# kokkos/kokkos-kernels

Measured on AMD Instinct MI355X. Metric: SpMV GFLOP/s (CSR, 27-pt 3-D FE Laplacian, fp64), higher is better.
Workload: dtype f64

## Files before the change

### kokkos-kernels_amd/csrc/kk_spmv.hip

```cpp
#include "kk_common.h"
#include "kk_scan.h"
#include <new>
#include <cstring>
#include <climits>

#include "kk_spmv_plan.h"

namespace kk {

template <class OffT, class AT, class YT, int LPR>
__global__ __launch_bounds__(kBlock) void spmv_vector_kernel(int64_t nrows, const OffT* __restrict__ row_map,
                                                             const int32_t* __restrict__ entries,
                                                             const AT* __restrict__ values, const YT* __restrict__ x,
                                                             YT* __restrict__ y, YT alpha, YT beta, int remap) {
  constexpr int RPB = kBlock / LPR;
  const int64_t wg  = remap ? xcd_remap(blockIdx.x, gridDim.x) : (int64_t)blockIdx.x;
  const int64_t row = wg * RPB + threadIdx.x / LPR;
  const int lane    = threadIdx.x % LPR;
  YT sum            = YT(0);
  if (row < nrows) {
    const OffT s = row_map[row], e = row_map[row + 1];
    for (OffT j = s + lane; j < e; j += LPR) sum += (YT)values[j] * x[entries[j]];
  }
  sum = group_sum(sum, LPR);
// ... 134 lines not shown
  uint16_t* out = wcode + s + (int64_t)t * NPT;
  if constexpr (NPT % 8 == 0) {
    KK_UNROLL
    for (int k = 0; k < NPT; k += 8) {
      kk_u32x4 v;
      v[0] = code[k] | (code[k + 1] << 16); v[1] = code[k + 2] | (code[k + 3] << 16);
      v[2] = code[k + 4] | (code[k + 5] << 16); v[3] = code[k + 6] | (code[k + 7] << 16);
      *reinterpret_cast<kk_u32x4*>(out + k) = v;
    }
  } else {
    KK_UNROLL
    for (int k = 0; k < NPT; k += 2) *reinterpret_cast<unsigned*>(out + k) = code[k] | (code[k + 1] << 16);
  }
  if (t == 0) {
    int off = 0;
    for (int w = 0; w < kWinCount; ++w) { s_off[w] = off; off += 64 * s_nch[w]; }
    s_off[kWinCount] = off;
    constexpr int CAP = TILE < kWinChunks * 64 ? TILE : kWinChunks * 64;
    const int mode = (off > CAP || !allow_stage) ? kTileCodes : kTileStaged;
    tinfo[b] = mode;
  }
  __syncthreads();
  int32_t* meta = wmeta + b * kWinMeta;
  if (t < kWinCount) { meta[t] = s_base[t]; meta[kWinCount + t] = s_off[t]; }
  if (t < kWinChunks) {
    const int slot = t * 64;
    int col = -1;
    for (int w = 0; w < kWinCount; ++w) if (slot >= s_off[w] && slot < s_off[w] + 64 * s_nch[w]) col = s_base[w] + (slot - s_off[w]);
    meta[2 * kWinCount + t] = col;
  }
}

constexpr int kPatSeg = 8, kPatLen = 32, kPatRec = 8, kPatTab = kPatRec + 4 * kPatSeg, kPatW = kPatTab + kPatSeg * kPatLen / 2;

template <class OffT, int NPT>
__global__ __launch_bounds__(kBlock) void pat_build_kernel(int64_t nnz, const OffT* __restrict__ row_map,
                                                           const int32_t* __restrict__ blk_info,
                                                           const uint16_t* __restrict__ wcode, const int32_t* __restrict__ wmeta,
                                                           int32_t* __restrict__ tinfo, int32_t* __restrict__ pmeta) {
  constexpr int TILE = kBlock * NPT, STEPS = NPT / 2, SPAN = kBlock * 2;
  __shared__ unsigned short s_slot[TILE];
  __shared__ unsigned char s_head[TILE + 2];
  __shared__ int s_segq[kPatSeg];
  __shared__ int s_nseg, s_bad, s_chunks;
  const int t = threadIdx.x;
  const int64_t b = blockIdx.x, s = b * TILE;
  int32_t* out = pmeta + b * kPatW;
  if ((tinfo[b] & 3) != kTileStaged) return;
  if (t == 0) { s_nseg = 0; s_bad = (s + TILE <= nnz) ? 0 : 1; s_chunks = 0; }
  __syncthreads();
  const int ldsoff = wmeta[b * kWinMeta + kWinCount + (t & (kWinCount - 1))];
  KK_UNROLL
  for (int k = 0; k < STEPS; ++k) {
    KK_UNROLL
    for (int j = 0; j < 2; ++j) {
      const unsigned code = wcode[s + (int64_t)t * NPT + 2 * k + j];
      const int off = __shfl(ldsoff, (int)(code >> kWinBits), 64);
      s_slot[k * SPAN + 2 * t + j] = (unsigned short)(off + (int)(code & ((1u << kWinBits) - 1)));
    }
  }
  if (t < kWinChunks && wmeta[b * kWinMeta + 2 * kWinCount + t] >= 0) atomicAdd(&s_chunks, 1);
  const int32_t info0 = blk_info[b], info1 = blk_info[b + 1];
  const int64_t ra = info0 & 0x7fffffff, rb = info1 & 0x7fffffff;
  const int has_head = (info0 >> 31) & 1;
  const int64_t nv = (rb - ra) + has_head;
  __syncthreads();
// ... 2 lines not shown
    const int64_t r  = ra + q - has_head;
    const int64_t rs = (int64_t)row_map[r] - s, re = (int64_t)row_map[r + 1] - s, L = re - rs;
    bool head = true;
    if (L < 1 || L > kPatLen) atomicOr(&s_bad, 1);
    else if (q > 0) {
      const int64_t ps = (int64_t)row_map[r - 1] - s;
      if (rs - ps == L) {
        head = false;
        for (int k = 0; k < (int)L; ++k) {
          const int64_t i0 = ps + k, i1 = rs + k;
          if (i0 >= 0 && i1 < TILE && (int)s_slot[i1] != (int)s_slot[i0] + 1) head = true;
        }
      }
    }
    s_head[q] = head ? 1 : 0;
    if (head) { const int idx = atomicAdd(&s_nseg, 1); if (idx < kPatSeg) s_segq[idx] = (int)q; }
  }
  __syncthreads();
  const int nseg = s_nseg;
  if (s_bad || nseg > kPatSeg || nseg < 1) return;
  if (t == 0) {
    for (int a = 1; a < nseg; ++a) { const int v = s_segq[a]; int c = a - 1; while (c >= 0 && s_segq[c] > v) { s_segq[c + 1] = s_segq[c]; --c; } s_segq[c + 1] = v; }
  }
  __syncthreads();
  if (t < kPatSeg) {
    int sb = INT_MAX, rs32 = 0, L32 = 1; float M = 1.0f;
    if (t < nseg) {
      const int64_t r  = ra + s_segq[t] - has_head;
      const int64_t rs = (int64_t)row_map[r] - s, L = (int64_t)row_map[r + 1] - s - rs;
      sb = rs > 0 ? (int)rs : 0; rs32 = (int)rs; L32 = (int)L;
      M  = 1.0f / (float)L;
    }
    if (t >= 1) out[t] = sb;
    out[kPatRec + 4 * t + 0] = sb; out[kPatRec + 4 * t + 1] = -rs32; out[kPatRec + 4 * t + 2] = L32; out[kPatRec + 4 * t + 3] = __float_as_int(M);
  }
  if (t == 0) { out[0] = nseg; tinfo[b] = kTilePattern; }
  if (t < kPatSeg * kPatLen) {
    const int g = t / kPatLen, k = t % kPatLen;
    int val = 0;
    if (g < nseg) {
      const int q = s_segq[g];
      const int64_t r  = ra + q - has_head;
      const int64_t rs = (int64_t)row_map[r] - s, re = (int64_t)row_map[r + 1] - s;
      if (k < re - rs) {
        const int64_t i = rs + k;
        if (i >= 0 && i < TILE) val = (int)s_slot[i];
        else if (i < 0 && q + 1 < nv && !s_head[q + 1] && re + k < TILE) val = (int)s_slot[re + k] - 1;
      }
    }
    reinterpret_cast<short*>(out + kPatTab)[t] = (short)val;
  }
}

template <class OffT, int NPT>
__global__ __launch_bounds__(kBlock) void pat_direct_kernel(int64_t nnz, const OffT* __restrict__ row_map, const int32_t* __restrict__ entries,
                                                            const int32_t* __restrict__ blk_info, int32_t* __restrict__ wmeta,
                                                            int32_t* __restrict__ tinfo, int32_t* __restrict__ pmeta) {
  constexpr int TILE = kBlock * NPT, NI = kPatSeg * kPatLen;
  static_assert(NI == kBlock, "one interval per work-item");
  __shared__ int s_col[TILE];
  __shared__ int s_segq[kPatSeg];
  __shared__ int s_lo[NI], s_hi[NI];
  __shared__ int s_base[kWinCount], s_nch[kWinCount], s_off[kWinCount + 1];
  __shared__ int s_nseg, s_bad;
  const int t = threadIdx.x, lane = t & 63, wave = t >> 6;
  const int64_t b = blockIdx.x, s = b * TILE;
  int32_t* out = pmeta + b * kPatW;
// ... 89 lines not shown
      bool unc = false;
      KK_UNROLL
      for (int u = 0; u < NI / 64; ++u) unc |= ((long long)ihi[u] >= bound);
      failed = __ballot(unc) != 0ull;
      if (!failed && lane == 0) {
        for (int q = wn; q < kWinCount; ++q) { s_base[q] = q ? s_base[q - 1] : 0; s_nch[q] = 0; }
        int off = 0;
        for (int w = 0; w < kWinCount; ++w) { s_off[w] = off; off += 64 * s_nch[w]; }
        s_off[kWinCount] = off;
      }
    }
    if (lane == 0 && failed) s_bad = 1;
  }
  __syncthreads();
  constexpr int CAP = TILE < kWinChunks * 64 ? TILE : kWinChunks * 64;
  if (s_bad || s_off[kWinCount] > CAP || s_off[kWinCount] > TILE - kPatW) { if (t == 0) tinfo[b] = kTilePlain; return; }
  int32_t* meta = wmeta + b * kWinMeta;
  if (t < kWinCount) { meta[t] = s_base[t]; meta[kWinCount + t] = s_off[t]; }
  if (t < kWinChunks) {
    const int slot = t * 64;
    int col = -1;
    for (int w = 0; w < kWinCount; ++w) if (slot >= s_off[w] && slot < s_off[w] + 64 * s_nch[w]) col = s_base[w] + (slot - s_off[w]);
    meta[2 * kWinCount + t] = col;
  }
  if (t < kPatSeg) {
    int sb = INT_MAX, rs32 = 0, L32 = 1; float M = 1.0f;
    if (t < nseg) {
      const int64_t r  = ra + s_segq[t] - has_head;
      const int64_t rs = (int64_t)row_map[r] - s, L = (int64_t)row_map[r + 1] - s - rs;
      sb = rs > 0 ? (int)rs : 0; rs32 = (int)rs; L32 = (int)L;
      M  = 1.0f / (float)L;
    }
    if (t >= 1) out[t] = sb;
    out[kPatRec + 4 * t + 0] = sb; out[kPatRec + 4 * t + 1] = -rs32; out[kPatRec + 4 * t + 2] = L32; out[kPatRec + 4 * t + 3] = __float_as_int(M);
  }
  if (t == 0) { out[0] = nseg; tinfo[b] = kTilePattern; }
  {
    int val = 0;
    if (csrc >= 0) {
      for (int w = 0; w < kWinCount; ++w) if (s_nch[w] > 0 && csrc >= s_base[w] && csrc < s_base[w] + 64 * s_nch[w]) val = s_off[w] + (csrc - s_base[w]);
      val += cadj;
    }
    reinterpret_cast<short*>(out + kPatTab)[t] = (short)val;
  }
}

__global__ __launch_bounds__(kBlock) void tile_mode_hist_kernel(int64_t nblocks, const int32_t* __restrict__ tinfo, int* __restrict__ counts) {
  __shared__ int s_c[4];
  const int t = threadIdx.x;
  if (t < 4) s_c[t] = 0;
  __syncthreads();
  const int64_t b = (int64_t)blockIdx.x * kBlock + t;
  const int mode = b < nblocks ? (tinfo[b] & 3) : -1;
  for (int m = 0; m < 4; ++m) {
    const int c = __popcll(__ballot(mode == m));
    if ((t & 63) == 0 && c) atomicAdd(&s_c[m], c);
  }
  __syncthreads();
  if (t < 4 && s_c[t]) atomicAdd(counts + t, s_c[t]);
}

__global__ void code_flag_kernel(int64_t nblocks, int32_t* __restrict__ tinfo, int32_t* __restrict__ flag, int use_pat) {
  const int64_t b = (int64_t)blockIdx.x * blockDim.x + threadIdx.x;
  if (b > nblocks) return;
  if (b == nblocks) { flag[b] = 0; return; }
  int mode = tinfo[b] & 3;
  if (mode == kTilePattern && !use_pat) { mode = kTileStaged; tinfo[b] = mode; }
// ... 224 lines not shown
  YT x0[STEPS], x1[STEPS];
  KK_UNROLL
  for (int k = 0; k < STEPS; ++k) {
    x0[k] = (FULL || c0[k] >= 0) ? x[FULL ? c0[k] : (c0[k] >= 0 ? c0[k] : 0)] : YT(0);
    x1[k] = (FULL || c1[k] >= 0) ? x[FULL ? c1[k] : (c1[k] >= 0 ? c1[k] : 0)] : YT(0);
  }
  KK_UNROLL
  for (int k = 0; k < STEPS; ++k) {
    const int li = k * SPAN + t * 2;
    prod[li]     = (YT)v0[k] * x0[k];
    prod[li + 1] = (YT)v1[k] * x1[k];
  }
}

template <class YT> __device__ __forceinline__ YT strided_lds_sum(const YT* prod, int i0, int i1, int lane, int G) {
  YT s0 = YT(0), s1 = YT(0), s2 = YT(0), s3 = YT(0);
  int i = i0 + lane;
  const int G2 = 2 * G, G3 = 3 * G, G4 = 4 * G;
  for (; i + G3 < i1; i += G4) {
    const YT a = prod[i], b = prod[i + G], c = prod[i + G2], d = prod[i + G3];
    s0 += a; s1 += b; s2 += c; s3 += d;
  }
  for (; i < i1; i += G) s0 += prod[i];
  return (s0 + s1) + (s2 + s3);
}

template <class OffT, class AT, class YT, int NPT, int MODE>
__global__ __launch_bounds__(kBlock) void spmv_stream3_kernel(int64_t nnz, const OffT* __restrict__ row_map,
                                                              const int32_t* __restrict__ entries,
                                                              const AT* __restrict__ values, const YT* __restrict__ x,
                                                              YT* __restrict__ y, YT alpha, YT beta,
                                                              const int32_t* __restrict__ blk_info,
                                                              YT* __restrict__ carry_head, YT* __restrict__ carry_tail,
                                                              int remap, const int32_t* __restrict__ list,
                                                              const int32_t* __restrict__ tinfo,
                                                              const uint16_t* __restrict__ wcode,
                                                              const int32_t* __restrict__ wmeta, int64_t ncols,
                                                              const int32_t* __restrict__ pmeta KK_ABL_PARAM) {
  constexpr int TILE  = kBlock * NPT;
  constexpr int STEPS = NPT / 2;
  __shared__ YT prod[TILE];
  constexpr bool NT = false;
  const int t       = threadIdx.x;
  const int64_t pos = xcd_order(blockIdx.x, gridDim.x, remap);
  const int64_t b   = list ? (int64_t)list[pos] : pos;
  const int64_t s = b * TILE;
  const bool full = (s + TILE <= nnz);
  const int64_t e = full ? s + TILE : nnz;

  const int32_t info0 = blk_info[b], info1 = blk_info[b + 1];
  const uint16_t* wtile = nullptr;
  if (MODE == kTileCodes || MODE == kTileStaged) wtile = wcode + (int64_t)((unsigned)tinfo[b] >> 2) * TILE;

  AT v0[STEPS], v1[STEPS];
  int c0[STEPS], c1[STEPS];
  if (MODE >= kTileStaged) {
  } else if (MODE == kTileCodes) {
    if (full) load_tile_win<AT, STEPS, true>(values, wtile, wmeta, b, s, e, t, v0, v1, c0, c1);
    else      load_tile_win<AT, STEPS, false>(values, wtile, wmeta, b, s, e, t, v0, v1, c0, c1);
  } else {
    if (full) load_tile<AT, STEPS, NT, true>(values, entries, s, e, t, v0, v1, c0, c1);
    else      load_tile<AT, STEPS, NT, false>(values, entries, s, e, t, v0, v1, c0, c1);
  }

  const int64_t ra    = info0 & 0x7fffffff;
  const int64_t rb    = info1 & 0x7fffffff;
  const int has_head  = (info0 >> 31) & 1;
  const int64_t nv    = (rb - ra) + has_head;
  int G = 1;
  while (G < kWave && nv * (G * 2) <= kBlock) G *= 2;
  const int lane = t & (G - 1), grp = t / G, ngrp = kBlock / G;
  bool valid = grp < nv;
  int64_t r  = ra + grp - has_head;
  int64_t rs = 0, re = 0;
  if (valid) {
    if (KK_ABL(16)) { rs = s + (int64_t)grp * 27; re = rs + 27; }
    else { rs = (int64_t)row_map[r]; re = (int64_t)row_map[r + 1]; }
  }
  YT yold = YT(0);
  if (beta != YT(0) && valid && lane == 0 && r >= 0) yold = y[r];

  if (MODE == kTilePattern) {
    stage_products_win<AT, YT, STEPS, true, NT, true>(values, wtile, wmeta, x, ncols, prod, b, s, e, t, pmeta);
  } else if (MODE == kTileStaged) {
    if (full) stage_products_win<AT, YT, STEPS, true, NT, false>(values, wtile, wmeta, x, ncols, prod, b, s, e, t, nullptr);
    else      stage_products_win<AT, YT, STEPS, false, NT, false>(values, wtile, wmeta, x, ncols, prod, b, s, e, t, nullptr);
  } else {
    if (full) stage_products<AT, YT, STEPS, true, true>(x, prod, t, v0, v1, c0, c1);
    else      stage_products<AT, YT, STEPS, false, false>(x, prod, t, v0, v1, c0, c1);
  }
  if (!KK_ABL(32)) __syncthreads();

  for (int64_t base = 0; base < nv; base += ngrp) {
    if (base > 0) {
      valid = (base + grp) < nv;
      r     = ra + base + grp - has_head;
      if (valid) { rs = (int64_t)row_map[r]; re = (int64_t)row_map[r + 1]; }
    }
    const bool is_head  = r < ra;
    const bool complete = !is_head && re <= e;
    const int i0 = (int)((rs > s ? rs : s) - s), i1 = (int)((re < e ? re : e) - s);
    YT sum = valid ? (KK_ABL(8) ? prod[i0 < TILE ? i0 : 0] : strided_lds_sum<YT>(prod, i0, i1, lane, G)) : YT(0);
    sum = group_sum(sum, G);
    if (valid && lane == 0) {
      if (is_head) carry_head[b] = sum;
      else if (!complete) carry_tail[b] = sum;
      else if (!KK_ABL(4) && !(KK_ABL(64) && (b & 7))) {
        sum *= alpha;
        const YT out = (beta == YT(0)) ? sum : beta * (base == 0 ? yold : y[r]) + sum;
        y[KK_ABL(128) ? (r & 255) : r] = out;
      }
    }
  }
}

template <class OffT, class YT>
__global__ void spmv_stream_fixup_kernel(int64_t nblocks, int64_t nnz, int64_t tile, const OffT* __restrict__ row_map,
                                         const int32_t* __restrict__ blk_row, const YT* __restrict__ carry_head,
                                         const YT* __restrict__ carry_tail, YT* __restrict__ y, YT alpha, YT beta) {
  const int64_t b = (int64_t)blockIdx.x * blockDim.x + threadIdx.x;
  if (b >= nblocks) return;
  const int64_t ra = blk_row[b] & 0x7fffffff, rb = blk_row[b + 1] & 0x7fffffff;
  if (rb == ra) return;
  const int64_t e  = ((b + 1) * tile < nnz) ? (b + 1) * tile : nnz;
  const int64_t R  = rb - 1;
  const int64_t re = (int64_t)row_map[R + 1];
  if (re <= e) return;
  YT total = carry_tail[b];
  for (int64_t b2 = b + 1; b2 < nblocks && b2 * tile < re; ++b2) total += carry_head[b2];
  total *= alpha;
  y[R] = (beta == YT(0)) ? total : beta * y[R] + total;
}

template <class OffT, class AT, class YT, int LPR>
// ... 16 lines not shown
  int l = 1;
  while (l < 64 && l * 2 <= avg) l *= 2;
  return l;
}

template <class OffT, class AT, class YT, int LPR>
static int launch_vector(const kkamd_crs_t* A, const YT* x, YT* y, YT alpha, YT beta, int remap, hipStream_t st) {
  const int64_t nwg = ceil_div(A->num_rows, kBlock / LPR);
  KK_LAUNCH((spmv_vector_kernel<OffT, AT, YT, LPR>), (unsigned)nwg, kBlock, 0, st, A->num_rows,
            (const OffT*)A->d_row_map, (const int32_t*)A->d_entries, (const AT*)A->d_values, x, y, alpha, beta, remap);
  KK_LAUNCH_CHECK();
  return KKAMD_OK;
}

template <class OffT, class AT, class YT>
static int run_vector(const kkamd_crs_t* A, const YT* x, YT* y, YT alpha, YT beta, const SpmvTuning& tn, hipStream_t st) {
  const int remap = tn.xcd_remap == 1;
  switch (pick_lpr(A->num_rows, A->nnz, tn.lanes_per_row)) {
    case 1:  return launch_vector<OffT, AT, YT, 1>(A, x, y, alpha, beta, remap, st);
    case 2:  return launch_vector<OffT, AT, YT, 2>(A, x, y, alpha, beta, remap, st);
    case 4:  return launch_vector<OffT, AT, YT, 4>(A, x, y, alpha, beta, remap, st);
    case 8:  return launch_vector<OffT, AT, YT, 8>(A, x, y, alpha, beta, remap, st);
    case 16: return launch_vector<OffT, AT, YT, 16>(A, x, y, alpha, beta, remap, st);
    case 32: return launch_vector<OffT, AT, YT, 32>(A, x, y, alpha, beta, remap, st);
    default: return launch_vector<OffT, AT, YT, 64>(A, x, y, alpha, beta, remap, st);
  }
}

template <class OffT, class AT, class YT, int NPT>
static int launch_stream(const kkamd_spmv_plan* p, const kkamd_crs_t* A, const YT* x, YT* y, YT alpha, YT beta,
                         hipStream_t st) {
  YT* ch = reinterpret_cast<YT*>(p->d_carry);
  YT* ct = reinterpret_cast<YT*>(reinterpret_cast<char*>(p->d_carry) + 8 * p->nblocks);
#define KK_STREAM3(MODE, NTILES, LIST)                                                                                    \
  KK_LAUNCH((spmv_stream3_kernel<OffT, AT, YT, NPT, MODE>), (unsigned)(NTILES), kBlock, KK_LDS_PAD(p), st, A->nnz,        \
            (const OffT*)A->d_row_map, (const int32_t*)A->d_entries, (const AT*)A->d_values, x, y, alpha, beta,          \
            (const int32_t*)p->d_blk_row, ch, ct, p->tune.xcd_remap, (const int32_t*)(LIST), (const int32_t*)p->d_tinfo, \
            (const uint16_t*)p->d_wcode, (const int32_t*)p->d_wbase, A->num_cols, (const int32_t*)p->d_pmeta KK_ABL_ARG(p))
  if (!p->d_tinfo) {
    KK_STREAM3(kTilePlain, p->nblocks, nullptr);
  } else {
    if (NPT != 4 && p->n_mode[kTilePattern] > 0) KK_STREAM3((NPT == 4 ? kTileStaged : kTilePattern), p->n_mode[kTilePattern], p->d_list[kTilePattern]);
    if (p->n_mode[kTileStaged] > 0) KK_STREAM3(kTileStaged, p->n_mode[kTileStaged], p->d_list[kTileStaged]);
    if (p->n_mode[kTileCodes] > 0)  KK_STREAM3(kTileCodes, p->n_mode[kTileCodes], p->d_list[kTileCodes]);
    if (p->n_mode[kTilePlain] > 0)  KK_STREAM3(kTilePlain, p->n_mode[kTilePlain], p->d_list[kTilePlain]);
  }
#undef KK_STREAM3
  KK_LAUNCH_CHECK();
  KK_LAUNCH((spmv_stream_fixup_kernel<OffT, YT>), (unsigned)ceil_div(p->nblocks, kBlock), kBlock, 0, st, p->nblocks,
            A->nnz, (int64_t)p->tile, (const OffT*)A->d_row_map, (const int32_t*)p->d_blk_row, (const YT*)ch,
            (const YT*)ct, y, alpha, beta);
  KK_LAUNCH_CHECK();
  return KKAMD_OK;
}

template <class OffT, class AT, class YT>
static int run_stream(const kkamd_spmv_plan* p, const kkamd_crs_t* A, const YT* x, YT* y, YT alpha, YT beta, hipStream_t st) {
  const int npt = p->tile / kBlock;
  if (npt * kBlock != p->tile) return fail(KKAMD_ERR_STATE, "kkamd_spmv: plan tile %d is not a multiple of the workgroup size", p->tile);
  if (npt == 16) return launch_stream<OffT, AT, YT, 16>(p, A, x, y, alpha, beta, st);
  if (npt == 8)  return launch_stream<OffT, AT, YT, 8>(p, A, x, y, alpha, beta, st);
  if (npt == 4 && sizeof(AT) == 8) return launch_stream<OffT, AT, YT, (sizeof(AT) == 8 ? 4 : 8)>(p, A, x, y, alpha, beta, st);
  return fail(KKAMD_ERR_STATE, "kkamd_spmv: no kernel for %d nonzeros per work-item with %d-byte values", npt, (int)sizeof(AT));
}

template <class OffT, class AT, class YT>
static int run_transpose(const kkamd_crs_t* A, const YT* x, YT* y, YT alpha, YT beta, hipStream_t st) {
  int rc = launch_scale<YT>(y, A->num_cols, 1, 1, 1, beta, st);
  if (rc) return rc;
  const int64_t avg = A->nnz / A->num_rows;
  if (avg >= 32) {
    KK_LAUNCH((spmv_transpose_kernel<OffT, AT, YT, 32>), (unsigned)ceil_div(A->num_rows, kBlock / 32), kBlock, 0, st,
              A->num_rows, (const OffT*)A->d_row_map, (const int32_t*)A->d_entries, (const AT*)A->d_values, x, y, alpha);
  } else if (avg >= 6) {
    KK_LAUNCH((spmv_transpose_kernel<OffT, AT, YT, 8>), (unsigned)ceil_div(A->num_rows, kBlock / 8), kBlock, 0, st,
              A->num_rows, (const OffT*)A->d_row_map, (const int32_t*)A->d_entries, (const AT*)A->d_values, x, y, alpha);
  } else {
    KK_LAUNCH((spmv_transpose_kernel<OffT, AT, YT, 1>), (unsigned)ceil_div(A->num_rows, kBlock), kBlock, 0, st,
// ... 364 lines not shown
  else if (k == "pattern_direct") { if (value != 0 && value != 1) return bad("0 or 1"); t.pattern_direct = value; }
  else if (k == "pattern_codes_min_knnz") { if (value < 0) return bad("non-negative"); t.pattern_codes_min_knnz = value; }
  else if (k == "colslab") { if (value < 0 || value > 4) return bad("in 0..4"); t.colslab = value; }
  else if (k == "colslab_min_pct") { if (value < 0 || value > 100) return bad("in 0..100"); t.colslab_min_pct = value; }
  else if (k == "colslab_min_knnz") { if (value < 0) return bad("non-negative"); t.colslab_min_knnz = value; }
  else if (k == "colslab_shift") { if (value != 0 && (value < 2 || value > 30)) return bad("0 or in 2..30"); t.colslab_shift = value; }
  else if (k == "colslab_rate_pct") { if (value < 1 || value > 1000) return bad("in 1..1000"); t.colslab_rate_pct = value; }
  else if (k == "values_tracking") { if (value < 0 || value > 2) return bad("in 0..2"); t.values_tracking = value; }
  else if (k == "check_entries") { if (value != 0 && value != 1) return bad("0 or 1"); t.check_entries = value; }
  else if (k == "defer_rank1") { if (value != 0 && value != 1) return bad("0 or 1"); t.defer_rank1 = value; }
  else if (k == "colslab_const") { if (value != 0 && value != 1) return bad("0 or 1"); t.colslab_const = value; }
  else if (k == "transient_min_knnz") { if (value < 0) return bad("non-negative"); t.transient_min_knnz = value; }
  else if (k == "explicit_transpose") { if (value < 0 || value > 2) return bad("in 0..2"); t.explicit_transpose = value; }
  else if (k == "explicit_transpose_min_knnz") { if (value < 0) return bad("non-negative"); t.explicit_transpose_min_knnz = value; }
#ifdef KK_ABLATE
  else if (k == "ablate") t.ablate = value;
  else if (k == "lds_pad_kb") t.lds_pad_kb = value;
#endif
  else return fail(KKAMD_ERR_INVALID_ARG, "unknown tuning key '%s'", key);
  return KKAMD_OK;
}

template <class OffT>
static int analyse(kkamd_spmv_plan* p, const kkamd_crs_t* A, hipStream_t st) {
  KK_LAUNCH((spmv_plan_kernel<OffT>), (unsigned)ceil_div(p->nblocks + 1, kBlock), kBlock, 0, st, A->num_rows,
            (const OffT*)A->d_row_map, p->nblocks, (int64_t)p->tile, p->d_blk_row);
  KK_LAUNCH_CHECK();
  return KKAMD_OK;
}

static void free_analysis(kkamd_spmv_plan* p) {
  void** bufs[] = {(void**)&p->d_blk_row, &p->d_carry, (void**)&p->d_tinfo, (void**)&p->d_wcode, (void**)&p->d_wbase, (void**)&p->d_pmeta};
  for (void** b : bufs) if (*b) { (void)hipFree(*b); *b = nullptr; }
  for (int m = 0; m < 4; ++m) { if (p->d_list[m]) { (void)hipFree(p->d_list[m]); p->d_list[m] = nullptr; } p->n_mode[m] = 0; }
  p->pat_tiles = p->code_tiles = p->staged_tiles = p->plain_tiles = 0; p->pat_direct = false;
  p->tile = 0; p->nblocks = 0; p->plan_bytes = 0;
}

static int build_codes(kkamd_spmv_plan* p, const kkamd_crs_t* A, hipStream_t st, int npt, bool may_retile, int* redo_npt) {
  *redo_npt = 0;
  const size_t nb = (size_t)p->nblocks;
  DevBuf full, counts, flag, tinfo_b, wbase_b;
  auto give_up = [&]() {
    (void)hipGetLastError();
    if (p->d_pmeta) { (void)hipFree(p->d_pmeta); p->d_pmeta = nullptr; }
    if (p->d_wcode) { (void)hipFree(p->d_wcode); p->d_wcode = nullptr; }
    for (int m = 0; m < 4; ++m) { if (p->d_list[m]) { (void)hipFree(p->d_list[m]); p->d_list[m] = nullptr; } p->n_mode[m] = 0; }
    p->d_tinfo = nullptr; p->d_wbase = nullptr;
    p->pat_tiles = p->code_tiles = p->staged_tiles = 0; p->plain_tiles = p->nblocks;
    p->win_failed = true;
    return KKAMD_OK;
  };
  if (full.alloc(sizeof(uint16_t) * nb * (size_t)p->tile) != hipSuccess || counts.alloc(12 * sizeof(int)) != hipSuccess ||
      flag.alloc(sizeof(int32_t) * (nb + 1)) != hipSuccess || tinfo_b.alloc(sizeof(int32_t) * nb) != hipSuccess ||
      wbase_b.alloc(sizeof(int32_t) * nb * kWinMeta) != hipSuccess)
    return give_up();
  int32_t* tinfo = tinfo_b.as<int32_t>();
  int32_t* wbase = wbase_b.as<int32_t>();
  uint16_t* d_full = full.as<uint16_t>();
  int* d_counts    = counts.as<int>();
  int32_t* d_flag  = flag.as<int32_t>();
  KK_HIP(hipMemsetAsync(counts.p, 0, 12 * sizeof(int), st));
  const int allow_stage = p->tune.window_codes != 2;
  const int32_t* ent = (const int32_t*)p->entries;
  auto make_lists = [&](const int64_t* known, size_t* list_bytes) -> int {
    for (int m = 0; m < 4; ++m) {
      if (known && known[m] == 0) { p->n_mode[m] = 0; continue; }
      if (known && known[m] == (int64_t)nb) { p->n_mode[m] = (int64_t)nb; continue; }
      KK_LAUNCH(mode_flag_kernel, (unsigned)ceil_div((int64_t)nb + 1, kBlock), kBlock, 0, st, (int64_t)nb, (const int32_t*)tinfo, d_flag, m);
      if (hipGetLastError() != hipSuccess) return -1;
      int rc2 = exclusive_scan_inplace<int32_t>(d_flag, (int64_t)nb + 1, st);
      if (rc2) { give_up(); return rc2; }
      int32_t cnt = 0;
      if (known) cnt = (int32_t)known[m];
      else {
        KK_HIP(hipMemcpyAsync(&cnt, d_flag + nb, sizeof(int32_t), hipMemcpyDeviceToHost, st));
        KK_HIP(hipStreamSynchronize(st));
      }
      p->n_mode[m] = cnt;
      if (cnt > 0 && (size_t)cnt < nb) {
        if (hipMalloc((void**)&p->d_list[m], sizeof(int32_t) * (size_t)cnt) != hipSuccess) return -1;
        *list_bytes += sizeof(int32_t) * (size_t)cnt;
        int32_t* d_list_m = p->d_list[m];
        KK_LAUNCH(mode_scatter_kernel, (unsigned)ceil_div((int64_t)nb, kBlock), kBlock, 0, st, (int64_t)nb, (const int32_t*)tinfo, (const int32_t*)d_flag, d_list_m, m);
        if (hipGetLastError() != hipSuccess) return -1;
      }
    }
    return 0;
  };
  const bool pat_wanted = p->tune.pattern_codes && (npt == 16 || npt == 8) &&
                          (p->tune.pattern_codes >= 2 || A->nnz >= (int64_t)p->tune.pattern_codes_min_knnz * 1000);
  if (pat_wanted && allow_stage && p->tune.pattern_direct && hipMalloc((void**)&p->d_pmeta, sizeof(int32_t) * nb * kPatW) == hipSuccess) {
    const bool o64 = A->offset_type == KKAMD_I64;
    int* d_cnt = d_counts + 8;
#define KK_PAT_DIRECT(OT, N)                                                                                                 \
  KK_LAUNCH((pat_direct_kernel<OT, N>), (unsigned)nb, kBlock, 0, st, A->nnz, (const OT*)A->d_row_map, ent,                   \
            (const int32_t*)p->d_blk_row, wbase, tinfo, p->d_pmeta)
    if (npt == 16) { if (o64) { KK_PAT_DIRECT(int64_t, 16); } else { KK_PAT_DIRECT(int32_t, 16); } }
    else           { if (o64) { KK_PAT_DIRECT(int64_t, 8); } else { KK_PAT_DIRECT(int32_t, 8); } }
#undef KK_PAT_DIRECT
    if (hipGetLastError() != hipSuccess) return give_up();
    KK_LAUNCH(tile_mode_hist_kernel, (unsigned)ceil_div((int64_t)nb, kBlock), kBlock, 0, st, (int64_t)nb, (const int32_t*)tinfo, d_cnt);
    if (hipGetLastError() != hipSuccess) return give_up();
    int hd[4] = {0, 0, 0, 0};
    KK_HIP(hipMemcpyAsync(hd, d_cnt, 4 * sizeof(int), hipMemcpyDeviceToHost, st));
    KK_HIP(hipStreamSynchronize(st));
    const int64_t left = (int64_t)nb - hd[kTilePattern], allowed = (int64_t)nb / 100 > 1 ? (int64_t)nb / 100 : 1;
    if (hd[kTilePattern] > 0 && left <= allowed) {
      if (hipMalloc((void**)&p->d_wcode, sizeof(uint16_t) * (size_t)p->tile) != hipSuccess) return give_up();
      const int64_t known[4] = {left, 0, 0, (int64_t)hd[kTilePattern]};
      size_t list_bytes = 0;
      int rc2 = make_lists(known, &list_bytes);
      if (rc2) return rc2 == -1 ? give_up() : rc2;
      KK_HIP(hipStreamSynchronize(st));
      p->d_tinfo = (int32_t*)tinfo_b.release(); p->d_wbase = (int32_t*)wbase_b.release();
      p->plain_tiles = left; p->pat_tiles = hd[kTilePattern]; p->code_tiles = 0; p->staged_tiles = hd[kTilePattern]; p->pat_direct = true;
      p->plan_bytes += list_bytes + sizeof(int32_t) * nb * (1 + kWinMeta) + sizeof(uint16_t) * (size_t)p->tile + sizeof(int32_t) * nb * kPatW;
      return KKAMD_OK;
// ... 289 lines not shown
    kk::mv6_plan_destroy(plan->mv6); plan->mv6 = nullptr; plan->mv6_tried = false;
  }
  if (t.mv_long_T != old.mv_long_T && plan->mv_long_known) {
    if (plan->used) KK_HIP(hipStreamSynchronize(plan->last_stream));
    if (plan->d_mv_long) { KK_HIP(hipFree(plan->d_mv_long)); plan->d_mv_long = nullptr; }
    plan->mv_long_known = false; plan->n_mv_long = 0; plan->mv_long_T = 0; plan->mv_long_nnz = 0;
  }
  return KKAMD_OK;
}

int kkamd_spmv_plan_values_changed(kkamd_spmv_plan_t* plan) {
  if (!plan) return kk::fail(KKAMD_ERR_INVALID_ARG, "kkamd_spmv_plan_values_changed: null plan");
  plan->t_stale = true;
  kk::cs_mark_stale(plan->cs);
  return KKAMD_OK;
}

int kkamd_spmv_plan_query(const kkamd_spmv_plan_t* plan, const char* key, int64_t* value) {
  if (!plan || !key || !value) return kk::fail(KKAMD_ERR_INVALID_ARG, "kkamd_spmv_plan_query: null argument");
  const std::string k(key);
  if (k.rfind("transpose_plan_", 0) == 0) {
    if (!plan->t_plan) { *value = 0; return KKAMD_OK; }
    return kkamd_spmv_plan_query(plan->t_plan, k.c_str() + 15, value);
  }
  if (k == "tile") *value = plan->tile;
  else if (k == "tiles") *value = plan->nblocks;
  else if (k == "window_codes") *value = plan->d_tinfo ? 1 : 0;
  else if (k == "window_staged_x") *value = (plan->d_tinfo && plan->staged_tiles > 0) ? 1 : 0;
  else if (k == "plain_tiles") *value = plan->d_tinfo ? plan->plain_tiles : plan->nblocks;
  else if (k == "code_tiles") *value = plan->code_tiles;
  else if (k == "staged_tiles") *value = plan->d_tinfo ? plan->staged_tiles : 0;
  else if (k == "pattern_tiles") *value = plan->d_pmeta ? plan->pat_tiles : 0;
  else if (k == "plan_bytes") *value = (int64_t)plan->plan_bytes;
  else if (k == "transpose_bytes") {
    const int64_t ob = plan->offset_type == KKAMD_I64 ? 8 : 4, vb = plan->value_type == KKAMD_F64 ? 8 : 4;
    *value = plan->t_ready ? plan->nnz * (4 + ob + vb) + (plan->num_cols + 1) * ob + 16 * kk::values_fp_tiles(plan->nnz) + (plan->d_t_shadow ? plan->nnz * vb : 0) : 0;
  }
  else if (k == "transpose_cached") *value = plan->t_ready ? 1 : 0;
  else if (k == "mv_tiles") *value = kk::mv_plan_query(plan->mv, 0);
  else if (k == "mv_staged_tiles") *value = kk::mv_plan_query(plan->mv, 1);
  else if (k == "mv_long_rows") *value = plan->n_mv_long;
  else if (k == "mv_order") *value = plan->mv ? kk::mv_plan_query(plan->mv, 2) : (plan->d_mv2_order ? 2 : 0);
  else if (k == "mv_period") *value = plan->mv_period;
  else if (k == "mv_plan_bytes") *value = kk::mv_plan_query(plan->mv, 3) + kk::mv4_plan_query(plan->mv4, 3) + kk::mv5_plan_query(plan->mv5, 3) + kk::mv6_plan_query(plan->mv6, 2);
  else if (k == "mv4_workgroups") *value = kk::mv4_plan_query(plan->mv4, 0);
  else if (k == "mv4_other_rows") *value = kk::mv4_plan_query(plan->mv4, 1);
  else if (k == "mv4_stencil") *value = kk::mv4_plan_query(plan->mv4, 2);
  else if (k == "mv4_near_stride") *value = kk::mv4_plan_query(plan->mv4, 4);
  else if (k == "mv6_chunks") *value = kk::mv6_plan_query(plan->mv6, 0);
  else if (k == "mv6_empty_rows") *value = kk::mv6_plan_query(plan->mv6, 1);
  else if (k == "mv_long_nnz") *value = plan->mv_long_nnz;
  else if (k == "mv5_tiles") *value = kk::mv5_plan_query(plan->mv5, 0);
  else if (k == "mv5_other_rows") *value = kk::mv5_plan_query(plan->mv5, 1);
  else if (k == "mv5_blocks") *value = kk::mv5_plan_query(plan->mv5, 2);
  else if (k == "mv5_fill_permille") *value = kk::mv5_plan_query(plan->mv5, 4);
  else if (k == "pattern_direct") *value = plan->pat_direct ? 1 : 0;
  else if (k == "colslab") *value = plan->cs ? 1 : 0;
  else if (k == "colslab_tried") *value = plan->cs_tried ? 1 : 0;
  else if (k == "colslab_slabs") *value = kk::cs_plan_query(plan->cs, 0);
  else if (k == "colslab_shift") *value = kk::cs_plan_query(plan->cs, 1);
  else if (k == "colslab_bytes") *value = kk::cs_plan_query(plan->cs, 2);
  else if (k == "colslab_deterministic") *value = kk::cs_plan_query(plan->cs, 3);
  else if (k == "colslab_lines_permille") *value = (int64_t)(plan->cs_ratio * 1000.0 + 0.5);
  else if (k == "colslab_crs_us") *value = (int64_t)(plan->cs_crs_us + 0.5);
  else if (k == "colslab_us") *value = (int64_t)(plan->cs_us + 0.5);
  else if (k == "march_workgroups") *value = plan->tune.march ? kk::mv4_plan_query(plan->mv4, 5) : 0;
// ... 46 lines not shown
```

### kokkos-kernels_amd/csrc/kk_spmv_plan.h

```cpp
#pragma once
#include "kk_common.h"
#include <string>
#include <utility>
#include <vector>

#ifdef KK_ABLATE
#define KK_ABL_PARAM , int ablate
#define KK_ABL_ARG(p) , (p)->tune.ablate
#define KK_ABL(bit) ((ablate & (bit)) != 0)
#define KK_LDS_PAD(p) ((size_t)(p)->tune.lds_pad_kb * 1024)
#else
#define KK_ABL_PARAM
#define KK_ABL_ARG(p)
#define KK_ABL(bit) false
#define KK_LDS_PAD(p) ((size_t)0)
#endif

namespace kk {

struct SpmvTuning {
  int kernel         = 0;
  int lanes_per_row  = 0;
  int nnz_per_thread = 0;
  int xcd_remap      = 16;
// ... 47 lines not shown

}

constexpr int kTilePlain = 0, kTileCodes = 1, kTileStaged = 2, kTilePattern = 3;

struct kkamd_mv_plan;
struct kkamd_mv4_plan;
struct kkamd_cs_plan;
struct kkamd_mv5_plan;
struct kkamd_mv6_plan;

struct kkamd_spmv_plan {
  std::vector<std::pair<std::string, int>> set_log;
  int64_t num_rows = 0, num_cols = 0, nnz = 0;
  const void* row_map = nullptr;
  int offset_type = 0, value_type = 1, algorithm = 0;
  kk::SpmvTuning tune;
  int tile = 0;
  int64_t nblocks = 0;
  int num_cus = 256;
  int32_t* d_blk_row = nullptr;
  void* d_carry = nullptr;
  void* d_xpack = nullptr;
  size_t xpack_bytes = 0;
  void* d_ypack = nullptr;
  size_t ypack_bytes = 0;
  const void* entries = nullptr;
  int32_t* d_tinfo = nullptr;
  uint16_t* d_wcode = nullptr;
  int32_t* d_wbase = nullptr;
  int32_t* d_pmeta = nullptr;
  int32_t* d_list[4] = {nullptr, nullptr, nullptr, nullptr};
  int64_t n_mode[4]  = {0, 0, 0, 0};
  int64_t code_tiles = 0;
  int64_t staged_tiles = 0;
  int64_t pat_tiles = 0;
  bool pat_direct = false;
  int64_t plain_tiles = 0;
  size_t plan_bytes = 0;
  void* d_t_rm = nullptr; int32_t* d_t_ent = nullptr; void* d_t_perm = nullptr; void* d_t_val = nullptr; unsigned long long* d_t_fp = nullptr;
  kkamd_spmv_plan* t_plan = nullptr;
  void* d_t_shadow = nullptr;
  bool t_ready = false, t_failed = false, t_fp_valid = false, t_shadow_valid = false, t_shadow_failed = false, t_stale = true;
  bool rank1_deferred = false;
  bool win_failed = false;
  kkamd_mv_plan* mv = nullptr;
  bool mv_failed = false;
  kkamd_mv4_plan* mv4 = nullptr;
  bool mv4_tried = false;
  kkamd_mv5_plan* mv5 = nullptr;
  bool mv5_tried = false;
  kkamd_mv6_plan* mv6 = nullptr;
  bool mv6_tried = false;
  int32_t* d_mv2_order = nullptr;
  int32_t* d_mv_long = nullptr; int64_t n_mv_long = 0, mv_long_T = 0, mv_long_nnz = 0; bool mv_long_known = false;
  kkamd_cs_plan* cs = nullptr;
  bool cs_tried = false;
  double cs_crs_us = 0.0, cs_us = 0.0;
  double cs_ratio = 0.0;
  int mv2_rb = 0;
  bool mv2_tried = false, mv_period_known = false;
  int64_t mv_period = 0;
  hipStream_t last_stream = nullptr;
  bool used = false;
  unsigned long long entries_hash = 0; bool entries_hash_known = false;
};
// ... 78 lines not shown
```

Before: 1114.

## Derive pattern-tile row bounds from segment records and drop contiguous tile lists

In pattern tiles the stream kernel now loads the per-tile segment records as 16-byte words into registers and computes each row's start and end from the segment's first row index, start offset and uniform length. This replaces the per-row row_map loads. Separately, when a mode's tile list turns out to be one contiguous range, the plan stores the first tile index and frees the list, so the kernel skips the indirect list lookup. The cost is extra register pressure and a host synchronisation during plan building.

```diff
diff --git a/kokkos-kernels_amd/csrc/kk_spmv.hip b/kokkos-kernels_amd/csrc/kk_spmv.hip
--- a/kokkos-kernels_amd/csrc/kk_spmv.hip
+++ b/kokkos-kernels_amd/csrc/kk_spmv.hip
@@ -190,6 +190,7 @@
 }
 
 constexpr int kPatSeg = 8, kPatLen = 32, kPatRec = 8, kPatTab = kPatRec + 4 * kPatSeg, kPatW = kPatTab + kPatSeg * kPatLen / 2;
+static_assert(kPatW % 4 == 0 && kPatRec % 4 == 0, "the kernel reads a record's segment entries as 16-byte words");
 
 template <class OffT, int NPT>
 __global__ __launch_bounds__(kBlock) void pat_build_kernel(int64_t nnz, const OffT* __restrict__ row_map,
@@ -258,7 +259,7 @@
       M  = 1.0f / (float)L;
     }
     if (t >= 1) out[t] = sb;
-    out[kPatRec + 4 * t + 0] = sb; out[kPatRec + 4 * t + 1] = -rs32; out[kPatRec + 4 * t + 2] = L32; out[kPatRec + 4 * t + 3] = __float_as_int(M);
+    out[kPatRec + 4 * t + 0] = t < nseg ? s_segq[t] : INT_MAX; out[kPatRec + 4 * t + 1] = -rs32; out[kPatRec + 4 * t + 2] = L32; out[kPatRec + 4 * t + 3] = __float_as_int(M);
   }
   if (t == 0) { out[0] = nseg; tinfo[b] = kTilePattern; }
   if (t < kPatSeg * kPatLen) {
@@ -414,7 +415,7 @@
       M  = 1.0f / (float)L;
     }
     if (t >= 1) out[t] = sb;
-    out[kPatRec + 4 * t + 0] = sb; out[kPatRec + 4 * t + 1] = -rs32; out[kPatRec + 4 * t + 2] = L32; out[kPatRec + 4 * t + 3] = __float_as_int(M);
+    out[kPatRec + 4 * t + 0] = t < nseg ? s_segq[t] : INT_MAX; out[kPatRec + 4 * t + 1] = -rs32; out[kPatRec + 4 * t + 2] = L32; out[kPatRec + 4 * t + 3] = __float_as_int(M);
   }
   if (t == 0) { out[0] = nseg; tinfo[b] = kTilePattern; }
   {
@@ -705,7 +706,7 @@
                                                               YT* __restrict__ y, YT alpha, YT beta,
                                                               const int32_t* __restrict__ blk_info,
                                                               YT* __restrict__ carry_head, YT* __restrict__ carry_tail,
-                                                              int remap, const int32_t* __restrict__ list,
+                                                              int remap, const int32_t* __restrict__ list, int64_t first,
                                                               const int32_t* __restrict__ tinfo,
                                                               const uint16_t* __restrict__ wcode,
                                                               const int32_t* __restrict__ wmeta, int64_t ncols,
@@ -716,7 +717,7 @@
   constexpr bool NT = false;
   const int t       = threadIdx.x;
   const int64_t pos = xcd_order(blockIdx.x, gridDim.x, remap);
-  const int64_t b   = list ? (int64_t)list[pos] : pos;
+  const int64_t b   = list ? (int64_t)list[pos] : first + pos;
   const int64_t s = b * TILE;
   const bool full = (s + TILE <= nnz);
   const int64_t e = full ? s + TILE : nnz;
@@ -746,8 +747,22 @@
   bool valid = grp < nv;
   int64_t r  = ra + grp - has_head;
   int64_t rs = 0, re = 0;
+  int pq[kPatSeg], ps[kPatSeg], pl[kPatSeg];
+  if (MODE == kTilePattern) {
+    const kk_u32x4* pm = reinterpret_cast<const kk_u32x4*>(pmeta + b * kPatW + kPatRec);
+    KK_UNROLL
+    for (int g = 0; g < kPatSeg; ++g) { const kk_u32x4 v = pm[g]; pq[g] = (int)v[0]; ps[g] = -(int)v[1]; pl[g] = (int)v[2]; }
+  }
+  auto pat_bounds = [&](int q, int& rs32, int& re32) {
+    int q0 = 0, st = ps[0], L = pl[0];
+    KK_UNROLL
+    for (int g = 1; g < kPatSeg; ++g) { const bool in = q >= pq[g]; q0 = in ? pq[g] : q0; st = in ? ps[g] : st; L = in ? pl[g] : L; }
+    rs32 = st + (q - q0) * L; re32 = rs32 + L;
+  };
+  int prs = 0, pre = 0;
   if (valid) {
-    if (KK_ABL(16)) { rs = s + (int64_t)grp * 27; re = rs + 27; }
+    if (MODE == kTilePattern) pat_bounds(grp, prs, pre);
+    else if (KK_ABL(16)) { rs = s + (int64_t)grp * 27; re = rs + 27; }
     else { rs = (int64_t)row_map[r]; re = (int64_t)row_map[r + 1]; }
   }
   YT yold = YT(0);
@@ -768,11 +783,21 @@
     if (base > 0) {
       valid = (base + grp) < nv;
       r     = ra + base + grp - has_head;
-      if (valid) { rs = (int64_t)row_map[r]; re = (int64_t)row_map[r + 1]; }
+      if (valid) {
+        if (MODE == kTilePattern) pat_bounds((int)base + grp, prs, pre);
+        else { rs = (int64_t)row_map[r]; re = (int64_t)row_map[r + 1]; }
+      }
     }
     const bool is_head  = r < ra;
-    const bool complete = !is_head && re <= e;
-    const int i0 = (int)((rs > s ? rs : s) - s), i1 = (int)((re < e ? re : e) - s);
+    bool complete;
+    int i0, i1;
+    if (MODE == kTilePattern) {
+      complete = !is_head && pre <= TILE;
+      i0 = prs > 0 ? prs : 0; i1 = pre < TILE ? pre : TILE;
+    } else {
+      complete = !is_head && re <= e;
+      i0 = (int)((rs > s ? rs : s) - s); i1 = (int)((re < e ? re : e) - s);
+    }
     YT sum = valid ? (KK_ABL(8) ? prod[i0 < TILE ? i0 : 0] : strided_lds_sum<YT>(prod, i0, i1, lane, G)) : YT(0);
     sum = group_sum(sum, G);
     if (valid && lane == 0) {
@@ -855,18 +880,19 @@
                          hipStream_t st) {
   YT* ch = reinterpret_cast<YT*>(p->d_carry);
   YT* ct = reinterpret_cast<YT*>(reinterpret_cast<char*>(p->d_carry) + 8 * p->nblocks);
-#define KK_STREAM3(MODE, NTILES, LIST)                                                                                    \
+#define KK_STREAM3(MODE, NTILES, LIST, FIRST, ORDER)                                                                                    \
   KK_LAUNCH((spmv_stream3_kernel<OffT, AT, YT, NPT, MODE>), (unsigned)(NTILES), kBlock, KK_LDS_PAD(p), st, A->nnz,        \
             (const OffT*)A->d_row_map, (const int32_t*)A->d_entries, (const AT*)A->d_values, x, y, alpha, beta,          \
-            (const int32_t*)p->d_blk_row, ch, ct, p->tune.xcd_remap, (const int32_t*)(LIST), (const int32_t*)p->d_tinfo, \
+            (const int32_t*)p->d_blk_row, ch, ct, (ORDER), (const int32_t*)(LIST), (int64_t)(FIRST), (const int32_t*)p->d_tinfo, \
             (const uint16_t*)p->d_wcode, (const int32_t*)p->d_wbase, A->num_cols, (const int32_t*)p->d_pmeta KK_ABL_ARG(p))
   if (!p->d_tinfo) {
-    KK_STREAM3(kTilePlain, p->nblocks, nullptr);
+    KK_STREAM3(kTilePlain, p->nblocks, nullptr, 0, p->tune.xcd_remap);
   } else {
-    if (NPT != 4 && p->n_mode[kTilePattern] > 0) KK_STREAM3((NPT == 4 ? kTileStaged : kTilePattern), p->n_mode[kTilePattern], p->d_list[kTilePattern]);
-    if (p->n_mode[kTileStaged] > 0) KK_STREAM3(kTileStaged, p->n_mode[kTileStaged], p->d_list[kTileStaged]);
-    if (p->n_mode[kTileCodes] > 0)  KK_STREAM3(kTileCodes, p->n_mode[kTileCodes], p->d_list[kTileCodes]);
-    if (p->n_mode[kTilePlain] > 0)  KK_STREAM3(kTilePlain, p->n_mode[kTilePlain], p->d_list[kTilePlain]);
+    const int remap = p->tune.xcd_remap;
+    if (NPT != 4 && p->n_mode[kTilePattern] > 0) KK_STREAM3((NPT == 4 ? kTileStaged : kTilePattern), p->n_mode[kTilePattern], p->d_list[kTilePattern], p->mode_first[kTilePattern], remap);
+    if (p->n_mode[kTileStaged] > 0) KK_STREAM3(kTileStaged, p->n_mode[kTileStaged], p->d_list[kTileStaged], p->mode_first[kTileStaged], remap);
+    if (p->n_mode[kTileCodes] > 0)  KK_STREAM3(kTileCodes, p->n_mode[kTileCodes], p->d_list[kTileCodes], p->mode_first[kTileCodes], remap);
+    if (p->n_mode[kTilePlain] > 0)  KK_STREAM3(kTilePlain, p->n_mode[kTilePlain], p->d_list[kTilePlain], p->mode_first[kTilePlain], remap);
   }
 #undef KK_STREAM3
   KK_LAUNCH_CHECK();
@@ -1297,7 +1323,7 @@
 static void free_analysis(kkamd_spmv_plan* p) {
   void** bufs[] = {(void**)&p->d_blk_row, &p->d_carry, (void**)&p->d_tinfo, (void**)&p->d_wcode, (void**)&p->d_wbase, (void**)&p->d_pmeta};
   for (void** b : bufs) if (*b) { (void)hipFree(*b); *b = nullptr; }
-  for (int m = 0; m < 4; ++m) { if (p->d_list[m]) { (void)hipFree(p->d_list[m]); p->d_list[m] = nullptr; } p->n_mode[m] = 0; }
+  for (int m = 0; m < 4; ++m) { if (p->d_list[m]) { (void)hipFree(p->d_list[m]); p->d_list[m] = nullptr; } p->n_mode[m] = 0; p->mode_first[m] = 0; }
   p->pat_tiles = p->code_tiles = p->staged_tiles = p->plain_tiles = 0; p->pat_direct = false;
   p->tile = 0; p->nblocks = 0; p->plan_bytes = 0;
 }
@@ -1310,7 +1336,7 @@
     (void)hipGetLastError();
     if (p->d_pmeta) { (void)hipFree(p->d_pmeta); p->d_pmeta = nullptr; }
     if (p->d_wcode) { (void)hipFree(p->d_wcode); p->d_wcode = nullptr; }
-    for (int m = 0; m < 4; ++m) { if (p->d_list[m]) { (void)hipFree(p->d_list[m]); p->d_list[m] = nullptr; } p->n_mode[m] = 0; }
+    for (int m = 0; m < 4; ++m) { if (p->d_list[m]) { (void)hipFree(p->d_list[m]); p->d_list[m] = nullptr; } p->n_mode[m] = 0; p->mode_first[m] = 0; }
     p->d_tinfo = nullptr; p->d_wbase = nullptr;
     p->pat_tiles = p->code_tiles = p->staged_tiles = 0; p->plain_tiles = p->nblocks;
     p->win_failed = true;
@@ -1330,6 +1356,7 @@
   const int32_t* ent = (const int32_t*)p->entries;
   auto make_lists = [&](const int64_t* known, size_t* list_bytes) -> int {
     for (int m = 0; m < 4; ++m) {
+      p->mode_first[m] = 0;
       if (known && known[m] == 0) { p->n_mode[m] = 0; continue; }
       if (known && known[m] == (int64_t)nb) { p->n_mode[m] = (int64_t)nb; continue; }
       KK_LAUNCH(mode_flag_kernel, (unsigned)ceil_div((int64_t)nb + 1, kBlock), kBlock, 0, st, (int64_t)nb, (const int32_t*)tinfo, d_flag, m);
@@ -1349,6 +1376,15 @@
         int32_t* d_list_m = p->d_list[m];
         KK_LAUNCH(mode_scatter_kernel, (unsigned)ceil_div((int64_t)nb, kBlock), kBlock, 0, st, (int64_t)nb, (const int32_t*)tinfo, (const int32_t*)d_flag, d_list_m, m);
         if (hipGetLastError() != hipSuccess) return -1;
+        int32_t ends[2] = {0, 0};
+        KK_HIP(hipMemcpyAsync(&ends[0], d_list_m, sizeof(int32_t), hipMemcpyDeviceToHost, st));
+        KK_HIP(hipMemcpyAsync(&ends[1], d_list_m + (cnt - 1), sizeof(int32_t), hipMemcpyDeviceToHost, st));
+        KK_HIP(hipStreamSynchronize(st));
+        if ((int64_t)ends[1] - ends[0] + 1 == (int64_t)cnt) {
+          p->mode_first[m] = ends[0];
+          (void)hipFree(p->d_list[m]); p->d_list[m] = nullptr;
+          *list_bytes -= sizeof(int32_t) * (size_t)cnt;
+        }
       }
     }
     return 0;
@@ -1704,6 +1740,9 @@
   else if (k == "staged_tiles") *value = plan->d_tinfo ? plan->staged_tiles : 0;
   else if (k == "pattern_tiles") *value = plan->d_pmeta ? plan->pat_tiles : 0;
   else if (k == "plan_bytes") *value = (int64_t)plan->plan_bytes;
+  else if (k == "tile_lists") { *value = 0; for (int m = 0; m < 4; ++m) *value += plan->d_list[m] ? 1 : 0; }
+  else if (k == "pattern_list") *value = plan->d_list[kTilePattern] ? 1 : 0;
+  else if (k == "pattern_first_tile") *value = plan->mode_first[kTilePattern];
   else if (k == "transpose_bytes") {
     const int64_t ob = plan->offset_type == KKAMD_I64 ? 8 : 4, vb = plan->value_type == KKAMD_F64 ? 8 : 4;
     *value = plan->t_ready ? plan->nnz * (4 + ob + vb) + (plan->num_cols + 1) * ob + 16 * kk::values_fp_tiles(plan->nnz) + (plan->d_t_shadow ? plan->nnz * vb : 0) : 0;
diff --git a/kokkos-kernels_amd/csrc/kk_spmv_plan.h b/kokkos-kernels_amd/csrc/kk_spmv_plan.h
--- a/kokkos-kernels_amd/csrc/kk_spmv_plan.h
+++ b/kokkos-kernels_amd/csrc/kk_spmv_plan.h
@@ -103,6 +103,7 @@
   int32_t* d_pmeta = nullptr;
   int32_t* d_list[4] = {nullptr, nullptr, nullptr, nullptr};
   int64_t n_mode[4]  = {0, 0, 0, 0};
+  int64_t mode_first[4] = {0, 0, 0, 0};
   int64_t code_tiles = 0;
   int64_t staged_tiles = 0;
   int64_t pat_tiles = 0;
```

Measured after the change: 1118, median of 4. Within noise of the previous version (+0.4%).
